# stefanopini/simple-HRNet

Hardware: AMD Instinct MI355X
Metric: person-crops/sec HRNet-W48 384x288 (model forward + heat-map decode) (higher is better)
Workload: dtype bf16; 1 GPU; HRNet-W48 384x288, batch=256 random crops per GPU, bf16 MFMA (BASELINE configs[2]); global_batch=256, micro_batch=256, lanes_per_gpu=1, parallelism=dp1 (crop sharding, RCCL all-gather of keypoints), weights=random-init seeded (synth_state_dict seed 0), BN stats randomised, engine_switches=

## Files before the change

### include/hrnet_mi355.h

```cpp
#ifndef HRNET_MI355_H
#define HRNET_MI355_H

#include <stddef.h>
#include <stdint.h>

#ifdef __cplusplus
extern "C" {
#endif

typedef struct hrn_ctx *hrn_handle;

enum { HRN_F32 = 0, HRN_BF16 = 1, HRN_F16 = 2 };
enum { HRN_BOX_I32 = 0, HRN_BOX_F32 = 1 };
enum { HRN_T_F32 = 0, HRN_T_I64 = 1 };

typedef struct {
    const char *name;
    const void *data;
    int32_t ndim;
    int64_t dims[4];
    int32_t dtype;
} hrn_tensor_desc;

typedef struct {
// ... 168 lines not shown
int hrn_refine_coords(hrn_handle h, const float *heatmaps_dev, int n, int refine, float *coords_dev, void *stream);

int hrn_nms(int32_t *keep_out, int32_t *num_out, const float *boxes_host, int boxes_num, int boxes_dim,
            float nms_overlap_thresh, int device_id);
int hrn_nms_release(int device_id);
const char *hrn_nms_last_error(void);

int hrn_oks_nms(int32_t *keep_out, int32_t *num_out, const double *kpts, const double *areas, const int32_t *order, int n, int J,
                double thresh, const double *sigmas, double in_vis_thre);
int hrn_soft_oks_nms(int32_t *keep_out, int32_t *num_out, const double *kpts, const double *areas, const double *scores_sorted,
                     const int32_t *order, int n, int J, double thresh, const double *sigmas, double in_vis_thre);
int hrn_pose_similarity(const double *boxes_a, const float *poses_a, int na, const double *boxes_b, const float *poses_b, int nb, int J,
                        float *sim_bbox, float *sim_pose);
int hrn_assignment(const double *cost, int rows, int cols, int32_t *row_to_col);

typedef struct {
    char name[96];
    int32_t c, h, w;
    int32_t conv_index;
} hrn_tap_info;
int hrn_tap_count(hrn_handle h);
int hrn_get_tap_info(hrn_handle h, int index, hrn_tap_info *out);
int hrn_forward_tap(hrn_handle h, const void *images_dev, int n, const char *tap_name, int crop0, int ncrops, int crop_step,
                    float *dst_dev, float *heatmaps_dev, void *stream);

int hrn_conv_count(hrn_handle h);
int hrn_get_conv_info(hrn_handle h, int index, hrn_conv_info *out);
double hrn_flops_per_crop(hrn_handle h);
int64_t hrn_workspace_bytes(hrn_handle h);
int64_t hrn_map_rebuilds(hrn_handle h);
int hrn_launches_per_pass(hrn_handle h);
int hrn_stem_fused(hrn_handle h);
int hrn_conv_compact(hrn_handle h, int index);
const char *hrn_switches(hrn_handle h);
int64_t hrn_debug_pad_violations(hrn_handle h);
int hrn_plan_block_map(hrn_handle h, int group, int n, int reverse, int32_t *blocks, int capacity, int32_t *members,
                       int member_capacity);
int hrn_plan_direct_map(hrn_handle h, int group, int n, int32_t *blocks, int capacity, int32_t *members, int member_capacity,
                        int32_t *pixels_per_tile);
int hrn_plan_s2_map(hrn_handle h, int group, int n, int32_t *blocks, int capacity, int32_t *parts, int part_capacity,
                    int32_t *active);
int hrn_profile_pass(hrn_handle h, const void *images_dev, int n, float *conv_ms, int conv_ms_len,
                     float *other_ms , void *stream);
const char *hrn_version(void);

#ifdef __cplusplus
}
#endif
#endif
```

### simple-hrnet_amd/_lib.py

```python
from __future__ import annotations

import ctypes
import os
import shutil
import subprocess
from typing import List

_HERE = os.path.dirname(os.path.abspath(__file__))
CSRC = os.path.join(_HERE, "csrc")
INCLUDE = os.path.join(os.path.dirname(_HERE), "include")
LIB_PATH = os.path.join(_HERE, "libhrnet_mi355.so")
if os.environ.get("HRN_LIB_TAG"):
    LIB_PATH = LIB_PATH.replace(".so", "_%s.so" % os.environ["HRN_LIB_TAG"])
SOURCES = ["kernels.hip", "conv3x3_lds.hip", "conv_s2.hip", "stem_fused.hip", "conv3x3_f32.hip", "bottleneck_chain.hip", "prepath.hip", "warp.hip", "nms.hip", "postproc.cpp", "hrnet_mi355.cpp",
           "decode.hip",
           "score.hip",
           "draw.hip",
           "track.hip",
           "pose_nms.hip",
           "letterbox.hip",
           "assoc.hip",
           "conv3x3_lds_f16.hip", "conv_s2_f16.hip", "bottleneck_chain_f16.hip"]
HEADERS = [os.path.join(CSRC, "kernels.h"), os.path.join(CSRC, "dt16.h"), os.path.join(CSRC, "argmax.h"), os.path.join(CSRC, "conv3x3_n96.inc"), os.path.join(CSRC, "conv3x3_lds.inc"),
           os.path.join(CSRC, "conv_s2.inc"), os.path.join(CSRC, "bottleneck_chain.inc"), os.path.join(INCLUDE, "hrnet_mi355.h")]
# ... 208 lines not shown
    "hrn_crop_geometry": (ctypes.c_int, [_P, ctypes.c_int, ctypes.c_int, _P, ctypes.c_int, ctypes.c_int, ctypes.c_int, ctypes.c_int, _P, _P]),
    "hrn_crop_geometry_last_error": (ctypes.c_char_p, []),
    "hrn_pose_boxes": (ctypes.c_int, [_P, ctypes.c_int, ctypes.c_int, _P, ctypes.c_int, ctypes.c_float, ctypes.c_int, ctypes.c_double,
                                      ctypes.c_double, _P]),
    "hrn_pose_boxes_last_error": (ctypes.c_char_p, []),
    "hrn_boxes_from_poses": (ctypes.c_int, [_P, _P, ctypes.c_int, ctypes.c_int, _P, ctypes.c_int, ctypes.c_float, ctypes.c_int,
                                            ctypes.c_double, ctypes.c_double, _P, _P]),
    "hrn_preprocess_frames_dev": (ctypes.c_int, [_P, ctypes.POINTER(Frame), ctypes.c_int, _P, ctypes.c_int, _P, ctypes.c_int, ctypes.c_int,
                                                 _P, _P, _P, _P]),
    "hrn_preprocess_frames_yuv_dev": (ctypes.c_int, [_P, ctypes.POINTER(YuvFrameC), ctypes.c_int, _P, ctypes.c_int, _P, ctypes.c_int,
                                                     ctypes.c_int, _P, _P, _P, _P]),
    "hrn_forward_flip_tta": (ctypes.c_int, [_P, _P, ctypes.c_int, _P, ctypes.c_int, ctypes.c_int, _P, _P, _P, _P]),
    "hrn_forward_refined": (ctypes.c_int, [_P, _P, ctypes.c_int, _P, ctypes.c_int, ctypes.c_int, _P, _P, _P]),
    "hrn_refine_coords": (ctypes.c_int, [_P, _P, ctypes.c_int, ctypes.c_int, _P, _P]),
    "hrn_nms": (ctypes.c_int, [_P, _P, _P, ctypes.c_int, ctypes.c_int, ctypes.c_float, ctypes.c_int]),
    "hrn_nms_release": (ctypes.c_int, [ctypes.c_int]),
    "hrn_nms_last_error": (ctypes.c_char_p, []),
    "hrn_oks_nms": (ctypes.c_int, [_P, _P, _P, _P, _P, ctypes.c_int, ctypes.c_int, ctypes.c_double, _P, ctypes.c_double]),
    "hrn_soft_oks_nms": (ctypes.c_int, [_P, _P, _P, _P, _P, _P, ctypes.c_int, ctypes.c_int, ctypes.c_double, _P, ctypes.c_double]),
    "hrn_pose_similarity": (ctypes.c_int, [_P, _P, ctypes.c_int, _P, _P, ctypes.c_int, ctypes.c_int, _P, _P]),
    "hrn_assignment": (ctypes.c_int, [_P, ctypes.c_int, ctypes.c_int, _P]),
    "hrn_tap_count": (ctypes.c_int, [_P]),
    "hrn_get_tap_info": (ctypes.c_int, [_P, ctypes.c_int, ctypes.POINTER(TapInfo)]),
    "hrn_forward_tap": (ctypes.c_int, [_P, _P, ctypes.c_int, ctypes.c_char_p, ctypes.c_int, ctypes.c_int, ctypes.c_int, _P, _P, _P]),
    "hrn_conv_count": (ctypes.c_int, [_P]),
    "hrn_get_conv_info": (ctypes.c_int, [_P, ctypes.c_int, ctypes.POINTER(ConvInfo)]),
    "hrn_flops_per_crop": (ctypes.c_double, [_P]),
    "hrn_workspace_bytes": (ctypes.c_int64, [_P]),
    "hrn_map_rebuilds": (ctypes.c_int64, [_P]),
    "hrn_launches_per_pass": (ctypes.c_int, [_P]),
    "hrn_switches": (ctypes.c_char_p, [_P]),
    "hrn_stem_fused": (ctypes.c_int, [_P]),
    "hrn_conv_compact": (ctypes.c_int, [_P, ctypes.c_int]),
    "hrn_debug_pad_violations": (ctypes.c_int64, [_P]),
    "hrn_plan_block_map": (ctypes.c_int, [_P, ctypes.c_int, ctypes.c_int, ctypes.c_int, _P, ctypes.c_int, _P, ctypes.c_int]),
    "hrn_plan_direct_map": (ctypes.c_int, [_P, ctypes.c_int, ctypes.c_int, _P, ctypes.c_int, _P, ctypes.c_int, _P]),
    "hrn_plan_s2_map": (ctypes.c_int, [_P, ctypes.c_int, ctypes.c_int, _P, ctypes.c_int, _P, ctypes.c_int, _P]),
    "hrn_profile_pass": (ctypes.c_int, [_P, _P, ctypes.c_int, ctypes.POINTER(ctypes.c_float), ctypes.c_int,
                                        ctypes.POINTER(ctypes.c_float), _P]),
    "hrn_version": (ctypes.c_char_p, []),
}

_lib = None


def load(auto_build: bool = True) -> ctypes.CDLL:
    global _lib
    if _lib is not None:
        return _lib
    if auto_build and needs_build():
        build()
    lib = ctypes.CDLL(LIB_PATH)
    for name, (res, args) in SYMBOLS.items():
        fn = getattr(lib, name)
        fn.restype = res
        fn.argtypes = args
    _lib = lib
    return lib


def header_symbols() -> List[str]:
    import re

    text = open(os.path.join(INCLUDE, "hrnet_mi355.h")).read()
    text = re.sub(r"/\*.*?\*/", "", text, flags=re.S)
    return sorted(set(re.findall(r"\b(hrn_[a-z_0-9]+)\s*\(", text)))
# ... 1 lines not shown
```

### simple-hrnet_amd/csrc/ctx_memory.inc

```
    bool hip_ok(hipError_t e, const char *what) {
        if (e == hipSuccess) return true;
        err = std::string(what) + ": " + hipGetErrorString(e);
        return false;
    }
    bool refuse_plan_only() {
        if (plan_only) err = "plan-only handle (device_id < 0): there is no CPU compute path";
        return plan_only;
    }

    bool allocate() {
        workspace_bytes = 0;
        for (auto &b : buffers) workspace_bytes += (int64_t)b.bytes;
        const int64_t small_crops = std::min<int64_t>(max_batch, (191 + head_slabs) / head_slabs);
        const int64_t part = std::max((int64_t)max_batch * joints * head_slabs, small_crops * joints * head_slabs_small);
        workspace_bytes += part * 8;
        if (plan_only) {
            fill_problems();
            index_s2groups();
            blob = (char *)calloc(1, (size_t)blob_bytes);
            return blob != nullptr;
        }
        if (!hip_ok(hipSetDevice(device), "hipSetDevice")) return false;
        for (auto &b : buffers) {
            if (!hip_ok(hipMalloc((void **)&b.dev, b.bytes), "hipMalloc(activation)")) return false;
// ... 110 lines not shown
                            ents.push_back({key, int2{prob | (nt << 8) | (tiles << 16), mt0 | (fused ? 1 << 29 : small_conv(cv) ? 1 << 30 : 0)}, bm});
                        }
            }
        }
        std::stable_sort(ents.begin(), ents.end(), [](const Ent &a, const Ent &b) { return a.key < b.key; });
        if (tile_px_out) {
            tile_px_out->resize(ents.size());
            for (size_t i = 0; i < ents.size(); ++i) (*tile_px_out)[i] = ents[i].bm;
        }
        if (out) {
            out->resize(ents.size());
            for (size_t i = 0; i < ents.size(); ++i) (*out)[i] = ents[i].v;
        }
        return (int)ents.size();
    }

    const Tensor &grid_of(const ConvOp &cv) const { return tensors[cv.up ? cv.in_t : cv.out_t]; }

    ConvArgs conv_args(const ConvOp &cv, int nb, bool rev) const {
        const Tensor &ti = tensors[cv.in_t], &to = grid_of(cv);
        ConvArgs a;
        a.in = row0(cv.in_t), a.out = row0(cv.out_t);
        a.w = blob + cv.w_off, a.bias = (const float *)(blob + cv.b_off);
        a.res = cv.res_t >= 0 ? row0(cv.res_t) : nullptr;
        a.cin = cv.cin, a.cout = cv.cout;
        a.in_wp = ti.wp, a.in_hpwp = ti.hpwp;
        a.out_h = to.h, a.out_w = to.w, a.out_wp = to.wp, a.out_hpwp = to.hpwp;
        a.m = nb * to.hpwp;
        a.ksize = cv.k, a.stride = cv.stride, a.relu = cv.relu, a.kchunks = cv.kchunks;
        a.rev = rev;
        a.pre_mode = pre_mode;
        a.wlds = direct_wlds && is16() ? 1 : 0;
        a.xlds = conv_xl(cv) ? 1 : 0;
        a.up = cv.up ? 1 : 0, a.up_a = cv.up ? (cv.up - 1) >> 1 : 0, a.up_b = cv.up ? (cv.up - 1) & 1 : 0;
        a.up_wp = tensors[cv.out_t].wp, a.up_hpwp = tensors[cv.out_t].hpwp;
        for (int t = 0; t < 4; ++t) {
            const int dy = (t >> 1) - 1 + a.up_a, dx = (t & 1) - 1 + a.up_b;
            a.taps[t] = cv.up ? dy * ti.wp + dx : 0;
        }
        return a;
    }

    int direct_group_blocks(const DirectGroup &g, int nb, std::vector<int2> *out, int mr = 4) const {
        struct Cls {
            int in_t, k, stride;
            std::vector<int> members;
            double cost = 0;
        };
        std::vector<Cls> cls;
        for (size_t k = 0; k < g.conv_idx.size(); ++k) {
            const ConvOp &cv = convs[g.conv_idx[k]];
            size_t ci = 0;
            for (; ci < cls.size(); ++ci)
                if (cls[ci].in_t == cv.in_t && cls[ci].k == cv.k && cls[ci].stride == cv.stride) break;
            if (ci == cls.size()) cls.push_back(Cls{cv.in_t, cv.k, cv.stride, {}, 0});
            cls[ci].members.push_back((int)k);
            cls[ci].cost += (double)grid_of(cv).hpwp * (cv.cout / (16 * g.nr)) * cv.kchunks;
        }
        std::stable_sort(cls.begin(), cls.end(), [](const Cls &a, const Cls &b) { return a.cost > b.cost; });
        int n = 0;
        if (out) out->clear();
        for (const Cls &cl : cls) {
            const int mtiles = (nb * grid_of(convs[g.conv_idx[cl.members[0]]]).hpwp + 64 * mr - 1) / (64 * mr);
            for (int round = 0; round * 8 < mtiles; ++round)
                for (int k : cl.members) {
                    const int ngroups = convs[g.conv_idx[k]].cout / (16 * g.nr);
// ... 297 lines not shown
```

### simple-hrnet_amd/csrc/ctx_run.inc

```
    struct Timing {
        std::vector<hipEvent_t> ev;
    };

    bool run_pass(const float *images, int nb, const void *boxes, int box_dtype, float *pts, float *heatmaps,
                  hipStream_t s, Timing *tm, int flip = 0, const TapReq *tap = nullptr, int refine = RF_NONE) {
        if (tm && !hip_ok(hipEventRecord(tm->ev[0], s), "hipEventRecord")) return false;
        const bool fused_stem = stem_fuse && !(tap && tap->op == 0);
        for (size_t oi = 0; oi < ops.size(); ++oi) {
            const bool rev = alternate && (oi & 1);
            hipError_t e = hipSuccess;
            if (fused_stem && oi == 0)
                e = exec_stem_fused(images, nb, s, flip);
            else if (!(fused_stem && (int)oi == stem_conv2_op))
                e = exec_op(ops[oi], rev, images, nb, boxes, box_dtype, pts, heatmaps, s, flip, refine);
            if (!hip_ok(e, "kernel launch")) return false;
            if (tap && tap->op == (int)oi) {
                const Tensor &t = tensors[tap->tensor];
                TapArgs a;
                a.in = row0(tap->tensor), a.dst = tap->dst;
                a.c = t.c, a.h = t.h, a.w = t.w, a.wp = t.wp, a.hpwp = t.hpwp;
                a.crop0 = tap->crop0, a.ncrops = tap->ncrops, a.crop_step = tap->crop_step;
                if (!hip_ok(launch_tap(dtype, a, s), "tap launch")) return false;
            }
            if (tm && !hip_ok(hipEventRecord(tm->ev[oi + 1], s), "hipEventRecord")) return false;
        }
        return true;
    }

    hipError_t exec_stem_fused(const float *images, int nb, hipStream_t s, int flip) {
        S2Group &g = stemf;
        bool hit;
        MapSlot *sl = find_slot(g.slot, nb, &hit);
        hipError_t e = slot_ready(sl, hit, s);
        if (e != hipSuccess) return e;
        if (!hit) {
            sl->nblocks = s2_blocks(g, nb, &g.map_host);
            if (sl->nblocks > g.map_capacity) return hipErrorInvalidValue;
            memcpy(sl->pin, g.map_host.data(), (size_t)sl->nblocks * sizeof(int2));
            e = hipMemcpyAsync(sl->dev, sl->pin, (size_t)sl->nblocks * sizeof(int2), hipMemcpyHostToDevice, s);
            if (e == hipSuccess) e = hipEventRecord(sl->landed, s);
// ... 22 lines not shown
            a.w = (const float *)(blob + stem_w_off), a.bias = (const float *)(blob + stem_b_off);
            a.wp = (is16() && !disable_stem_mfma) ? (const void *)(blob + stem_wp_off) : nullptr;
            a.n = nb, a.H = H, a.W = W;
            a.out_h = t.h, a.out_w = t.w, a.out_wp = t.wp, a.out_hpwp = t.hpwp;
            a.flip = flip;
            e = launch_stem(dtype, a, s);
            break;
        }
        case OP_STEM7: {
            const Tensor &t = tensors[stem_out_t];
            Stem7Args a;
            a.images = images, a.out = row0(stem_out_t);
            a.w = (const float *)(blob + stem_w_off), a.bias = (const float *)(blob + stem_b_off);
            a.wp = (is16() && !disable_stem_mfma) ? (const void *)(blob + stem_wp_off) : nullptr;
            a.n = nb, a.H = H, a.W = W;
            a.out_h = t.h, a.out_w = t.w, a.out_wp = t.wp, a.out_hpwp = t.hpwp;
            a.flip = flip;
            e = launch_stem7(dtype, a, s);
            break;
        }
        case OP_MAXPOOL: {
            const Tensor &ti = tensors[pool_in_t], &to = tensors[pool_out_t];
            PoolArgs a;
            a.in = row0(pool_in_t), a.out = row0(pool_out_t);
            a.c = to.c, a.n = nb, a.in_wp = ti.wp, a.in_hpwp = ti.hpwp;
            a.out_h = to.h, a.out_w = to.w, a.out_wp = to.wp, a.out_hpwp = to.hpwp;
            e = launch_maxpool(dtype, a, s);
            break;
        }
        case OP_CONV: {
            const ConvOp &cv = convs[op.idx];
            const ConvArgs a = conv_args(cv, nb, rev);
            e = launch_conv(dtype, a, cv.nr, s);
            break;
        }
        case OP_CONV3_GROUP: {
            Conv3Group &g = groups[op.idx];
            bool hit;
            MapSlot *sl = find_slot(g.slot, nb, &hit);
            if ((e = slot_ready(sl, hit, s)) != hipSuccess) break;
            if (!hit) {
                sl->nblocks = group_blocks(g, nb, &g.map_host, rev);
                if (sl->nblocks > g.map_capacity) {
                    e = hipErrorInvalidValue;
                    break;
                }
                memcpy(sl->pin, g.map_host.data(), (size_t)sl->nblocks * sizeof(int2));
                e = hipMemcpyAsync(sl->dev, sl->pin, (size_t)sl->nblocks * sizeof(int2), hipMemcpyHostToDevice, s);
                if (e == hipSuccess) e = hipEventRecord(sl->landed, s);
                if (e != hipSuccess) break;
                sl->nb = nb;
                ++map_builds;
            }
            e = (dtype == HRN_F16 ? launch_conv3x3_lds_f16 : launch_conv3x3_lds)(probs_dev + g.prob_first, sl->dev, sl->nblocks, nb,
                                                                             convs[g.conv_idx[0]].ks, convs[g.conv_idx[0]].nr, s);
            break;
        }
        case OP_CONV_GROUP: {
            DirectGroup &g = dgroups[op.idx];
            bool hit;
            MapSlot *sl = find_slot(g.slot, nb, &hit);
            if ((e = slot_ready(sl, hit, s)) != hipSuccess) break;
            if (!hit) {
                for (size_t k = 0; k < g.conv_idx.size(); ++k) sl->args_pin[k] = conv_args(convs[g.conv_idx[k]], nb, rev);
                sl->mr = 4;
                while (sl->mr > 1 && direct_group_blocks(g, nb, nullptr, sl->mr) < 512) sl->mr >>= 1;
// ... 146 lines not shown
```

### simple-hrnet_amd/csrc/hrnet_mi355.cpp

```cpp
#include "../../include/hrnet_mi355.h"

#include <hip/hip_runtime.h>

#include <algorithm>
#include <cmath>
#include <cstdio>
#include <cstdlib>
#include <cstring>
#include <map>
#include <memory>
#include <string>
#include <vector>

#include "assoc_math.h"
#include "letterbox_math.h"
#include "pose_nms_math.h"
#include "kernels.h"
#include "track_geometry.h"

namespace {
#include "ctx_types.h"
}

namespace {
// ... 30 lines not shown
    struct Chain {
        int conv3, conv1, ds;
        int conv2 = -1;
    };
    std::vector<Chain> chains;
    std::vector<TapPoint> taps;
    Conv3Problem *probs_dev = nullptr;
    std::vector<Op> ops;
    int stem_out_t = -1, head_in_t = -1;
    int64_t stem_w_off = 0, stem_b_off = 0, stem_wp_off = 0, head_w_off = 0, head_b_off = 0, head_wp_off = 0;

    int64_t blob_bytes = 0;
    char *blob = nullptr;
    bool weights_loaded = false;

    bool disable_lds = env_sw("HRN_DISABLE_LDS") != nullptr;
    bool assoc_no_assign = env_sw("HRN_ASSOC_NO_ASSIGN") != nullptr;
    bool disable_group = env_sw("HRN_DISABLE_GROUP") != nullptr;
    bool disable_dgroup = env_sw("HRN_DISABLE_DGROUP") != nullptr;
    bool disable_chain = env_sw("HRN_DISABLE_CHAIN") != nullptr;
    bool small_tiles = env_sw("HRN_SMALL_TILES") ? atoi(env_sw("HRN_SMALL_TILES")) != 0 : true;
    int small_below = env_sw("HRN_SMALL_BELOW") ? atoi(env_sw("HRN_SMALL_BELOW")) : 384;
    int small_keep_above = env_sw("HRN_SMALL_KEEP") ? atoi(env_sw("HRN_SMALL_KEEP")) : 300;
    bool disable_chain_ds = env_sw("HRN_DISABLE_CHAIN_DS") != nullptr;
    int pre_mode = env_sw("HRN_PRE_MODE") ? atoi(env_sw("HRN_PRE_MODE")) : 1;
    int chain_blocks = env_sw("HRN_CHAIN_BLOCKS") ? atoi(env_sw("HRN_CHAIN_BLOCKS")) : 512;
    bool disable_chain3 = env_sw("HRN_DISABLE_CHAIN3") != nullptr;
    bool direct_wlds = !(env_sw("HRN_DIRECT_WLDS") && atoi(env_sw("HRN_DIRECT_WLDS")) == 0);
    bool direct_xlds = !(env_sw("HRN_DIRECT_XLDS") && atoi(env_sw("HRN_DIRECT_XLDS")) == 0);
    bool conv_xl(const ConvOp &cv) const {
        return direct_xlds && direct_wlds && is16() && cv.k == 3 && cv.stride == 2 && cv.cin % 32 == 0 && !cv.up && cv.res_t < 0 && cv.nr == 6 &&
               cv.kchunks >= 4;
    }
    bool disable_bbf = env_sw("HRN_BBF") && atoi(env_sw("HRN_BBF")) == 0;
    int bbf_tpb_div = env_sw("HRN_BBF_TPB_DIV") ? std::max(1, atoi(env_sw("HRN_BBF_TPB_DIV"))) : 3;
    double bbf_slide_cost = env_sw("HRN_BBF_SLIDE_COST") ? atof(env_sw("HRN_BBF_SLIDE_COST")) : 24600.0;
    int bbf_min_tiles = env_sw("HRN_BBF_MIN_TILES") ? atoi(env_sw("HRN_BBF_MIN_TILES")) : 1100;
    int dgroup_nr_mode = env_sw("HRN_DGROUP_NR") ? atoi(env_sw("HRN_DGROUP_NR")) : 1;
    bool disable_lds32 = env_sw("HRN_DISABLE_LDS32") != nullptr;
    bool disable_n96 = env_sw("HRN_DISABLE_N96") != nullptr;
    bool disable_fgroup = env_sw("HRN_DISABLE_FGROUP") != nullptr;
    bool disable_f32lds = env_sw("HRN_DISABLE_F32LDS") != nullptr;
    int f32_small_slices = env_sw("HRN_F32_SMALL_SLICES") ? atoi(env_sw("HRN_F32_SMALL_SLICES")) : 0;
    std::vector<Conv3Problem> probs_host;
    bool disable_compact = env_sw("HRN_DISABLE_COMPACT") != nullptr;
    double compact_min_pad = env_sw("HRN_COMPACT_MIN_PAD") ? atof(env_sw("HRN_COMPACT_MIN_PAD")) : 0.08;
    bool disable_s2 = env_sw("HRN_DISABLE_S2") != nullptr;
    int s2_min_tiles = env_sw("HRN_S2_MIN_TILES") ? atoi(env_sw("HRN_S2_MIN_TILES")) : 256;
    int s2_target_blocks = env_sw("HRN_S2_BLOCKS") ? std::max(1, atoi(env_sw("HRN_S2_BLOCKS"))) : 256;
    bool disable_stem_mfma = env_sw("HRN_DISABLE_STEM_MFMA") != nullptr;
    bool disable_stem_fuse = env_sw("HRN_DISABLE_STEM_FUSE") != nullptr;
    bool stem_fuse = false;
    int stem_conv2_op = -1;
    S2Group stemf;
    bool disable_head_mfma = env_sw("HRN_DISABLE_HEAD_MFMA") != nullptr;
    bool direct_nr6 = env_sw("HRN_DIRECT_NR6") ? atoi(env_sw("HRN_DIRECT_NR6")) != 0 : true;
    int half_stages_per_block = env_sw("HRN_HALF_STAGES") ? atoi(env_sw("HRN_HALF_STAGES")) : 8;
    bool alternate = env_sw("HRN_ALTERNATE") ? atoi(env_sw("HRN_ALTERNATE")) != 0 : true;
    int block_order = env_sw("HRN_BLOCK_ORDER") ? atoi(env_sw("HRN_BLOCK_ORDER")) : 1;
    int long_factor = env_sw("HRN_LONG_FACTOR") ? atoi(env_sw("HRN_LONG_FACTOR")) : 4;
    double long_share = env_sw("HRN_LONG_SHARE") ? atof(env_sw("HRN_LONG_SHARE")) : 0.85;
    int head_slabs = 1, head_slab_px = 1024;
    static constexpr int kHeadSlabPxSmall = 256;
    int head_slabs_small = 1;
    int head_px_for(int nb) const { return (long)nb * head_slabs >= 192 ? head_slab_px : kHeadSlabPxSmall; }
    int head_slabs_for(int nb) const { return (long)nb * head_slabs >= 192 ? head_slabs : head_slabs_small; }
// ... 1248 lines not shown
}

int hrn_conv_count(hrn_handle h) { return h ? (int)h->convs.size() : 0; }

int hrn_get_conv_info(hrn_handle h, int index, hrn_conv_info *out) {
    if (!h || !out || index < 0 || index >= (int)h->convs.size()) return 1;
    const ConvOp &cv = h->convs[index];
    memset(out, 0, sizeof *out);
    snprintf(out->name, sizeof out->name, "%s", cv.conv.c_str());
    out->cin = cv.cin, out->cout = cv.cout, out->ksize = cv.k, out->stride = cv.stride, out->relu = cv.relu;
    out->has_residual = cv.res_t >= 0;
    out->in_h = h->tensors[cv.in_t].h, out->in_w = h->tensors[cv.in_t].w;
    out->out_h = h->tensors[cv.out_t].h, out->out_w = h->tensors[cv.out_t].w;
    out->kpad = cv.kpad, out->nr = cv.nr, out->algo = cv.fuse_with >= 0 || cv.fused_away ? 2 : cv.n96 ? 3 : cv.s2 ? 4 : cv.algo, out->ks = cv.ks;
    out->w_offset = cv.w_off, out->w_bytes = cv.w_bytes, out->b_offset = cv.b_off;
    out->flops = cv.flops;
    return 0;
}

double hrn_flops_per_crop(hrn_handle h) {
    if (!h) return 0;
    double f = 2.0 * 64 * (h->model == 1 ? 147 : 27) * (h->H / 2) * (double)(h->W / 2);
    for (auto &cv : h->convs) f += cv.flops;
    f += 2.0 * h->joints * h->head_c * (h->H / 4) * (double)(h->W / 4);
    return f;
}

int64_t hrn_workspace_bytes(hrn_handle h) { return h ? h->workspace_bytes : 0; }
int64_t hrn_map_rebuilds(hrn_handle h) { return h ? h->map_builds : -1; }
int hrn_launches_per_pass(hrn_handle h) { return h ? (int)h->ops.size() - (h->stem_fuse ? 1 : 0) : 0; }
int hrn_stem_fused(hrn_handle h) { return h && h->stem_fuse ? 1 : 0; }
int hrn_conv_compact(hrn_handle h, int index) { return h && index >= 0 && index < (int)h->convs.size() && h->convs[index].compact ? 1 : 0; }
const char *hrn_switches(hrn_handle h) { return h ? h->switches.c_str() : ""; }

int64_t hrn_debug_pad_violations(hrn_handle h) {
    if (!h || h->plan_only) return -1;
    if (!h->hip_ok(hipSetDevice(h->device), "hipSetDevice")) return -1;
    unsigned long long *cnt = nullptr, host = 0;
    if (!h->hip_ok(hipMalloc((void **)&cnt, sizeof *cnt), "hipMalloc") || !h->hip_ok(hipMemset(cnt, 0, sizeof *cnt), "hipMemset")) return -1;
    bool ok = h->hip_ok(hipDeviceSynchronize(), "hipDeviceSynchronize");
    for (const Buffer &b : h->buffers) {
        if (!ok) break;
        PadCheckArgs a;
        a.buf = b.dev, a.count = cnt, a.rows = (long)b.rows, a.lead_rows = (long)b.lead_rows;
        a.c = b.c, a.h = b.h, a.w = b.w, a.wp = b.w + 1, a.hpwp = (b.h + 1) * (b.w + 1), a.nmax = h->max_batch;
        ok = h->hip_ok(launch_pad_check(h->dtype, a, nullptr), "pad check launch");
    }
    ok = ok && h->hip_ok(hipMemcpy(&host, cnt, sizeof host, hipMemcpyDeviceToHost), "hipMemcpy");
    (void)hipFree(cnt);
    return ok ? (int64_t)host : -1;
}

int hrn_plan_block_map(hrn_handle h, int group, int n, int reverse, int32_t *blocks, int capacity, int32_t *members, int member_capacity) {
    if (!h || n <= 0 || n > h->max_batch) return -1;
    if (group < 0 || group >= (int)h->groups.size()) return -1;
    const Conv3Group &g = h->groups[group];
    std::vector<int2> map;
    std::vector<int> px;
    const int nblocks = h->group_blocks(g, n, &map, reverse != 0, false, &px);
    for (int i = 0; i < nblocks && i < capacity; ++i) {
        const int x = map[i].x, y = map[i].y;
        int32_t *o = blocks + (size_t)i * 6;
        o[0] = x & 0xff, o[1] = (x >> 8) & 0xff, o[2] = x >> 16, o[3] = y & 0x1fffffff, o[4] = px[i],
        o[5] = ((y >> 29) & 1) | (((y >> 30) & 1) << 1);
    }
    int nm = 0;
// ... 121 lines not shown
```

### simple-hrnet_amd/csrc/kernels.h

```cpp
#pragma once
#include <hip/hip_runtime.h>
#include <stdint.h>

#include <atomic>
#include <cstdlib>
#include <cstring>

namespace hrn {

inline hipError_t set_dynamic_lds(const void *func, int bytes, std::atomic<unsigned long long> &done) {
    int dev = 0;
    hipError_t e = hipGetDevice(&dev);
    if (e != hipSuccess) return e;
    const unsigned long long bit = 1ull << (dev & 63);
    if (done.load(std::memory_order_acquire) & bit) return hipSuccess;
    e = hipFuncSetAttribute(func, hipFuncAttributeMaxDynamicSharedMemorySize, bytes);
    if (e == hipSuccess) done.fetch_or(bit, std::memory_order_release);
    return e;
}

inline const char *hrn_env(const char *name) {
    static const bool debug = [] {
        const char *v = getenv("HRN_DEBUG_ENV");
        return v && *v && strcmp(v, "0") != 0;
    }();
    return debug ? getenv(name) : nullptr;
}

enum { DT_F32 = 0, DT_BF16 = 1, DT_F16 = 2 };

struct ConvArgs {
    const void *in;
    void *out;
    const void *w;
    const float *bias;
    const void *res;
    int cin, cout;
    int in_wp, in_hpwp;
    int out_h, out_w, out_wp, out_hpwp;
    int m;
    int ksize, stride, relu;
    int kchunks;
    int rev;
    int pre_mode;
    int wlds;
    int xlds;
    int up, up_a, up_b, up_wp, up_hpwp;
    int taps[4];
};

struct Conv3Problem {
    const void *in;
    void *out;
    const void *w;
    const float *bias;
    const void *res;
    int cin, cout;
    int h, wd, wp, hpwp;
    int relu;
    int slices;
    int ntiles;
    int tiles_per_block;
    int bm;
    unsigned magic_hpwp, magic_wp;
    int shift_hpwp, shift_wp;
    const void *w2;
    const float *bias2;
    int n96;
    int compact, hw;
    unsigned magic_hw, magic_w;
    int shift_hw, shift_w;
    int slab_rows, slab_rows_small;
};
int conv3x3_n96_ch64();
int conv3x3_lds_bbf_ok(int wp);
int conv3x3_n96_max_rows();
int conv3x3_lds_bm(int ks, int nrb, int wp);
int conv3x3_f32_bm(int wp);
hipError_t launch_conv3x3_f32(const Conv3Problem *probs_dev, const void *blockmap_dev, int nblocks, int nb, int nrb, hipStream_t s);
// ... 312 lines not shown
    unsigned char pad[4];
    LetterboxFrame one;
    const LetterboxFrame *table;
    void *out;
};
hipError_t launch_letterbox(const LetterboxArgs &a, hipStream_t s);
struct DetFrame;
struct DetFilter;
struct DetArgs {
    int P, compact;
    const DetFrame *table;
    const float *dets;
    float *out;
    int *counts, *status;
};
hipError_t launch_detections_to_frame(const DetArgs &a, const DetFrame &one, const DetFilter &q, hipStream_t s);

struct TapArgs {
    const void *in;
    float *dst;
    int c, h, w, wp, hpwp, crop0, ncrops, crop_step;
};
hipError_t launch_tap(int dtype, const TapArgs &a, hipStream_t s);

struct PadCheckArgs {
    const void *buf;
    unsigned long long *count;
    long rows, lead_rows;
    int c, h, w, wp, hpwp, nmax;
};
hipError_t launch_pad_check(int dtype, const PadCheckArgs &a, hipStream_t s);

hipError_t launch_conv(int dtype, const ConvArgs &a, int nr, hipStream_t s);
hipError_t launch_conv_group(int dtype, const ConvArgs *probs_dev, const void *map_dev, int nblocks, int nr, int mr, int wlds,
                             hipStream_t s);
hipError_t launch_conv3x3_lds(const Conv3Problem *probs_dev, const void *blockmap_dev, int nblocks, int nb, int ks,
                              int nrb, hipStream_t s);
hipError_t launch_conv3x3_lds_f16(const Conv3Problem *probs_dev, const void *blockmap_dev, int nblocks, int nb, int ks,
                                  int nrb, hipStream_t s);
hipError_t launch_stem(int dtype, const StemArgs &a, hipStream_t s);
hipError_t launch_fuse(int dtype, const FuseArgs &a, hipStream_t s);
hipError_t launch_head(int dtype, const HeadArgs &a, hipStream_t s);

constexpr int kConvBlockRows = 704;

}
```

### simple-hrnet_amd/csrc/kernels.hip

```cpp
#include "kernels.h"
#include "argmax.h"
#include "dt16.h"
#include <stdlib.h>

namespace hrn {

typedef __attribute__((ext_vector_type(8))) __bf16 bf16x8;
typedef __attribute__((ext_vector_type(8))) short s16x8;
typedef __attribute__((ext_vector_type(4))) short s16x4;
typedef __attribute__((ext_vector_type(4))) float f32x4;

__device__ __forceinline__ float bf16_to_f32(unsigned short h) { return __uint_as_float(((unsigned)h) << 16); }
__device__ __forceinline__ unsigned short f32_to_bf16(float f) {
    unsigned u = __float_as_uint(f);
    u += 0x7fffu + ((u >> 16) & 1u);
    return (unsigned short)(u >> 16);
}

constexpr bool is16(int dt) { return dt != DT_F32; }

template <int DT>
struct Tr;
template <>
struct Tr<DT_BF16> {
// ... 328 lines not shown
    for (int i = 0; i < MR; ++i)
#pragma unroll
        for (int j = 0; j < NR; ++j) acc[i][j] = f32x4{0.f, 0.f, 0.f, 0.f};
    w_issue(0);
    px_issue(0);
    px_issue(1);
    for (int kc = 0; kc < kchunks; ++kc) {
        const int gi = kc / XL_G, c = kc - gi * XL_G;
        if (c == 0) {
            asm volatile("s_waitcnt vmcnt(%0)" ::"i"((XL_D - 1) * MR) : "memory");
            __builtin_amdgcn_s_barrier();
            w_issue(gi + 1);
        }
        px_issue(kc + XL_D - 1);
        asm volatile("s_waitcnt vmcnt(%0)" ::"i"((XL_D - 1) * MR + WOPS) : "memory");
        s16x8 a[MR], b[NR];
        const unsigned xa = xring + (kc % XL_D) * (MR * 1024) + lane16;
        const unsigned wa = lds0 + ((gi & 1) * NR * XL_G + c) * 1024 + lane16;
#pragma unroll
        for (int i = 0; i < MR; ++i) asm volatile("ds_read_b128 %0, %1 offset:%2" : "=v"(a[i]) : "v"(xa), "i"(i * 1024));
#pragma unroll
        for (int j = 0; j < NR; ++j) asm volatile("ds_read_b128 %0, %1 offset:%2" : "=v"(b[j]) : "v"(wa), "i"(j * XL_G * 1024));
        asm volatile("s_waitcnt lgkmcnt(0)" ::: "memory");
#pragma unroll
        for (int i = 0; i < MR; ++i)
#pragma unroll
            for (int j = 0; j < NR; ++j) acc[i][j] = mma<DT>(b[j], a[i], acc[i][j]);
    }
    asm volatile("s_waitcnt vmcnt(0)" ::: "memory");
    s16x8 rpre[1][1];
    conv_direct_epilogue<DT, NR, MR, false>(p, ng, m0, li, g, acc, rpre);
}

template <int DT, int NR, int MR, bool PRE, bool WL = false>
__global__ __launch_bounds__(256) void conv_direct_kernel(const ConvArgs p) {
    extern __shared__ __attribute__((aligned(16))) char smem_direct[];
    const int ngroups = p.cout / (16 * NR);
    const int ng = (blockIdx.x >> 3) % ngroups;
    const int mtile = (blockIdx.x / (8 * ngroups)) * 8 + (blockIdx.x & 7);
    if constexpr (WL && is16(DT) && NR == 6 && MR == 4 && !PRE) {
        if (p.xlds && conv_xl_ok(p)) {
            conv_direct_xl_body<DT, NR>(p, ng, mtile, smem_direct);
            return;
        }
    }
    conv_direct_body<DT, NR, MR, PRE, WL>(p, ng, mtile, smem_direct);
}

template <int DT, int NR, int MR, bool WL = false>
__global__ __launch_bounds__(256) void conv_direct_group_kernel(const ConvArgs *__restrict__ probs,
                                                                const int2 *__restrict__ map) {
    extern __shared__ __attribute__((aligned(16))) char smem_direct[];
    const int2 e = map[blockIdx.x];
    const int prob = __builtin_amdgcn_readfirstlane(e.x & 255), ng = __builtin_amdgcn_readfirstlane(e.x >> 8);
    const int mtile = __builtin_amdgcn_readfirstlane(e.y);
    const ConvArgs p = probs[prob];
    if constexpr (WL && is16(DT) && NR == 6 && MR == 4) {
        if (p.xlds && conv_xl_ok(p)) {
            conv_direct_xl_body<DT, NR>(p, ng, mtile, smem_direct);
            return;
        }
    }
    conv_direct_body<DT, NR, MR, false, WL>(p, ng, mtile, smem_direct);
}

template <int DT, int NR>
// ... 39 lines not shown
        if (nr == 3) return launch_conv_group_t<DT_F16, 3>(probs_dev, map, nblocks, mr, wlds, s);
        if (nr == 2) return launch_conv_group_t<DT_F16, 2>(probs_dev, map, nblocks, mr, wlds, s);
    } else {
        if (nr == 4) return launch_conv_group_t<DT_F32, 4>(probs_dev, map, nblocks, mr, wlds, s);
        if (nr == 3) return launch_conv_group_t<DT_F32, 3>(probs_dev, map, nblocks, mr, wlds, s);
        if (nr == 2) return launch_conv_group_t<DT_F32, 2>(probs_dev, map, nblocks, mr, wlds, s);
    }
    return hipErrorInvalidValue;
}

template <int DT, int NR, int MR, bool PRE>
static hipError_t launch_conv_tt(const ConvArgs &a, hipStream_t s) {
    const int mtiles = (a.m + 64 * MR - 1) / (64 * MR);
    dim3 grid(((mtiles + 7) / 8) * 8 * (a.cout / (16 * NR)));
    hipLaunchKernelGGL((conv_direct_kernel<DT, NR, MR, PRE>), grid, dim3(256), 0, s, a);
    return hipGetLastError();
}

template <int DT, int NR>
static hipError_t launch_conv_t(const ConvArgs &a, hipStream_t s) {
    if constexpr (is16(DT) && NR % 2 == 0) {
        const int pre_mode = a.pre_mode;
        if (a.res && a.ksize == 1 && pre_mode == 1) return launch_conv_tt<DT, NR, 4, true>(a, s);
        if (a.res && a.ksize == 1 && pre_mode == 2) return launch_conv_tt<DT, NR, 2, true>(a, s);
        if (a.res && a.ksize == 1 && pre_mode == 3) return launch_conv_tt<DT, NR, 2, false>(a, s);
    }
    const int ngroups = a.cout / (16 * NR);
    const long blocks4 = (long)((a.m + 255) / 256) * ngroups;
    if (blocks4 < 256) return launch_conv_tt<DT, NR, 1, false>(a, s);
    if (blocks4 < 512) return launch_conv_tt<DT, NR, 2, false>(a, s);
    if constexpr (is16(DT))
        if (a.wlds && a.kchunks >= 2 * WL_G) {
            const int mtiles = (a.m + 255) / 256;
            dim3 grid(((mtiles + 7) / 8) * 8 * (a.cout / (16 * NR)));
            const int lds = direct_lds_bytes<DT, NR>(a.xlds ? 2 : 1);
            static std::atomic<unsigned long long> lds_set{0};
            if (lds > 65536) {
                const hipError_t e = set_dynamic_lds((const void *)conv_direct_kernel<DT, NR, 4, false, true>, direct_lds_bytes<DT, NR>(2), lds_set);
                if (e != hipSuccess) return e;
            }
            hipLaunchKernelGGL((conv_direct_kernel<DT, NR, 4, false, true>), grid, dim3(256), lds, s, a);
            return hipGetLastError();
        }
    return launch_conv_tt<DT, NR, 4, false>(a, s);
}

hipError_t launch_conv(int dtype, const ConvArgs &a, int nr, hipStream_t s) {
    if (a.m <= 0) return hipSuccess;
    if (dtype == DT_BF16) {
        if (nr == 6) return launch_conv_t<DT_BF16, 6>(a, s);
        if (nr == 4) return launch_conv_t<DT_BF16, 4>(a, s);
        if (nr == 3) return launch_conv_t<DT_BF16, 3>(a, s);
        if (nr == 2) return launch_conv_t<DT_BF16, 2>(a, s);
    } else if (dtype == DT_F16) {
        if (nr == 6) return launch_conv_t<DT_F16, 6>(a, s);
        if (nr == 4) return launch_conv_t<DT_F16, 4>(a, s);
        if (nr == 3) return launch_conv_t<DT_F16, 3>(a, s);
        if (nr == 2) return launch_conv_t<DT_F16, 2>(a, s);
    } else {
        if (nr == 4) return launch_conv_t<DT_F32, 4>(a, s);
        if (nr == 3) return launch_conv_t<DT_F32, 3>(a, s);
        if (nr == 2) return launch_conv_t<DT_F32, 2>(a, s);
    }
    return hipErrorInvalidValue;
}

// ... 667 lines not shown
```

### simple-hrnet_amd/native.py

```python
from __future__ import annotations

import contextlib
import ctypes
import math
from typing import Dict, List, Optional, Sequence, Tuple, Union

import numpy as np
import torch

from . import _lib
from .frames import (PIX_FORMATS, YUV_MATRICES, YUV_RANGES, Frames, YuvFrame, _check_frame, _frame_kind, as_tensor,
                     device_tensor, frame_stack, host_array, host_bytes)
from .palettes import bgr_to_yuv_colors, embedded_palette, find_palette

DTYPES = {"fp32": 0, "f32": 0, "float32": 0, torch.float32: 0, "bf16": 1, "bfloat16": 1, torch.bfloat16: 1,
          "fp16": 2, "f16": 2, "float16": 2, "half": 2, torch.float16: 2}
DTYPE_NAMES = {0: "fp32", 1: "bf16", 2: "fp16"}
REFINE_MODES = {None: 0, "quarter": 1, "dark": 2}


def refine_code(refine) -> int:
    if not (refine is None or isinstance(refine, str)) or refine not in REFINE_MODES:
        raise ValueError("refine must be None, 'quarter' or 'dark', got %r" % (refine,))
    return REFINE_MODES[refine]
# ... 1000 lines not shown
        if info is None:
            raise KeyError("no tensor named %r is written by this plan" % name)
        dst = torch.empty((ncrops, info.c, info.h, info.w), dtype=torch.float32, device=x.device)
        h, w = self.resolution
        hm = torch.empty((n, self.nof_joints, h // 4, w // 4), dtype=torch.float32, device=x.device) if return_heatmaps else None
        self._launch("hrn_forward_tap", x.data_ptr(), n, name.encode(), int(crop0), int(ncrops), int(crop_step), dst.data_ptr(),
                     hm.data_ptr() if hm is not None else None)
        return (dst, hm) if return_heatmaps else dst

    def conv_infos(self) -> List[_lib.ConvInfo]:
        out = []
        for i in range(self._lib.hrn_conv_count(self._h)):
            ci = _lib.ConvInfo()
            rc = self._lib.hrn_get_conv_info(self._h, i, ctypes.byref(ci))
            self._check(rc, "hrn_get_conv_info")
            out.append(ci)
        return out

    def flops_per_crop(self) -> float:
        return float(self._lib.hrn_flops_per_crop(self._h))

    def workspace_bytes(self) -> int:
        return int(self._lib.hrn_workspace_bytes(self._h))

    def map_rebuilds(self) -> int:
        return int(self._lib.hrn_map_rebuilds(self._h))

    def launches_per_pass(self) -> int:
        return int(self._lib.hrn_launches_per_pass(self._h))

    def conv_compact(self, index: int) -> bool:
        return bool(self._lib.hrn_conv_compact(self._h, index))

    def stem_fused(self) -> bool:
        return bool(self._lib.hrn_stem_fused(self._h))

    def pad_violations(self) -> int:
        return int(self._lib.hrn_debug_pad_violations(self._h))

    def switches(self) -> str:
        return self._lib.hrn_switches(self._h).decode()

    def profile_pass(self, images: torch.Tensor):
        x = self._images_ptr(images)
        n = min(x.shape[0], self.max_batch)
        nconv = self._lib.hrn_conv_count(self._h)
        conv_ms = (ctypes.c_float * nconv)()
        other = (ctypes.c_float * 4)()
        self._launch("hrn_profile_pass", x.data_ptr(), n, conv_ms, nconv, other)
        return list(conv_ms), dict(zip(("stem", "fuse", "head", "decode"), list(other)))


class MultiDeviceHRNet:

    def __init__(self, devices: Sequence[int], c: int = 48, nof_joints: int = 17, resolution: Tuple[int, int] = (384, 288),
                 dtype="bf16", max_batch: int = 32, model_name: str = "HRNet"):
        from concurrent.futures import ThreadPoolExecutor

        if len(devices) < 1:
            raise ValueError("at least one device")
        self.devices = [int(d) for d in devices]
        self.nets = [NativeHRNet(c, nof_joints, resolution, dtype, max_batch=max_batch, device=d, model_name=model_name)
                     for d in self.devices]
        self.streams = [torch.cuda.Stream(torch.device("cuda", d)) for d in self.devices]
        self.pool = ThreadPoolExecutor(max_workers=len(self.devices), thread_name_prefix="hrn-dev")
        first = self.nets[0]
# ... 155 lines not shown
```

Before: 11790 crops/s.

## Add wide 512-thread direct conv kernel for stride-2 XL convs

Adds a direct-convolution kernel for stride-2 3x3 convs with cout divisible by 192. Each 512-thread block covers two channel groups, so each staged pixel tile feeds twice the output channels. Weights are double-buffered and a three-stage pixel ring is prefetched two stages ahead. It is on by default and can be disabled with an env switch. It adds counters and query APIs, and trades more LDS per block and lower occupancy for more input reuse.

New measurement: 11840 crops/s (median of 6 runs). Within noise of the previous version (+0.5%).

```diff
diff --git a/include/hrnet_mi355.h b/include/hrnet_mi355.h
--- a/include/hrnet_mi355.h
+++ b/include/hrnet_mi355.h
@@ -224,6 +224,9 @@
 int hrn_launches_per_pass(hrn_handle h);
 int hrn_stem_fused(hrn_handle h);
 int hrn_conv_compact(hrn_handle h, int index);
+int hrn_conv_xl_wide(hrn_handle h, int index);
+int hrn_conv_op_index(hrn_handle h, int index);
+int64_t hrn_xl_wide_launches(hrn_handle h);
 const char *hrn_switches(hrn_handle h);
 int64_t hrn_debug_pad_violations(hrn_handle h);
 int hrn_plan_block_map(hrn_handle h, int group, int n, int reverse, int32_t *blocks, int capacity, int32_t *members,
diff --git a/simple-hrnet_amd/_lib.py b/simple-hrnet_amd/_lib.py
--- a/simple-hrnet_amd/_lib.py
+++ b/simple-hrnet_amd/_lib.py
@@ -264,6 +264,9 @@
     "hrn_switches": (ctypes.c_char_p, [_P]),
     "hrn_stem_fused": (ctypes.c_int, [_P]),
     "hrn_conv_compact": (ctypes.c_int, [_P, ctypes.c_int]),
+    "hrn_conv_xl_wide": (ctypes.c_int, [_P, ctypes.c_int]),
+    "hrn_conv_op_index": (ctypes.c_int, [_P, ctypes.c_int]),
+    "hrn_xl_wide_launches": (ctypes.c_int64, [_P]),
     "hrn_debug_pad_violations": (ctypes.c_int64, [_P]),
     "hrn_plan_block_map": (ctypes.c_int, [_P, ctypes.c_int, ctypes.c_int, ctypes.c_int, _P, ctypes.c_int, _P, ctypes.c_int]),
     "hrn_plan_direct_map": (ctypes.c_int, [_P, ctypes.c_int, ctypes.c_int, _P, ctypes.c_int, _P, ctypes.c_int, _P]),
diff --git a/simple-hrnet_amd/csrc/ctx_memory.inc b/simple-hrnet_amd/csrc/ctx_memory.inc
--- a/simple-hrnet_amd/csrc/ctx_memory.inc
+++ b/simple-hrnet_amd/csrc/ctx_memory.inc
@@ -166,6 +166,7 @@
         a.pre_mode = pre_mode;
         a.wlds = direct_wlds && is16() ? 1 : 0;
         a.xlds = conv_xl(cv) ? 1 : 0;
+        a.xlw = conv_xlw(cv) ? 1 : 0;
         a.up = cv.up ? 1 : 0, a.up_a = cv.up ? (cv.up - 1) >> 1 : 0, a.up_b = cv.up ? (cv.up - 1) & 1 : 0;
         a.up_wp = tensors[cv.out_t].wp, a.up_hpwp = tensors[cv.out_t].hpwp;
         for (int t = 0; t < 4; ++t) {
diff --git a/simple-hrnet_amd/csrc/ctx_run.inc b/simple-hrnet_amd/csrc/ctx_run.inc
--- a/simple-hrnet_amd/csrc/ctx_run.inc
+++ b/simple-hrnet_amd/csrc/ctx_run.inc
@@ -6,6 +6,7 @@
                   hipStream_t s, Timing *tm, int flip = 0, const TapReq *tap = nullptr, int refine = RF_NONE) {
         if (tm && !hip_ok(hipEventRecord(tm->ev[0], s), "hipEventRecord")) return false;
         const bool fused_stem = stem_fuse && !(tap && tap->op == 0);
+        xlw_launches = 0;
         for (size_t oi = 0; oi < ops.size(); ++oi) {
             const bool rev = alternate && (oi & 1);
             hipError_t e = hipSuccess;
@@ -94,6 +95,7 @@
             const ConvOp &cv = convs[op.idx];
             const ConvArgs a = conv_args(cv, nb, rev);
             e = launch_conv(dtype, a, cv.nr, s);
+            if (conv_takes_xlw(a)) ++xlw_launches;
             break;
         }
         case OP_CONV3_GROUP: {
diff --git a/simple-hrnet_amd/csrc/hrnet_mi355.cpp b/simple-hrnet_amd/csrc/hrnet_mi355.cpp
--- a/simple-hrnet_amd/csrc/hrnet_mi355.cpp
+++ b/simple-hrnet_amd/csrc/hrnet_mi355.cpp
@@ -86,6 +86,9 @@
         return direct_xlds && direct_wlds && is16() && cv.k == 3 && cv.stride == 2 && cv.cin % 32 == 0 && !cv.up && cv.res_t < 0 && cv.nr == 6 &&
                cv.kchunks >= 4;
     }
+    bool direct_xlw = !(env_sw("HRN_DIRECT_XLW") && atoi(env_sw("HRN_DIRECT_XLW")) == 0);
+    bool conv_xlw(const ConvOp &cv) const { return direct_xlw && conv_xl(cv) && cv.cout % 192 == 0; }
+    int64_t xlw_launches = 0;
     bool disable_bbf = env_sw("HRN_BBF") && atoi(env_sw("HRN_BBF")) == 0;
     int bbf_tpb_div = env_sw("HRN_BBF_TPB_DIV") ? std::max(1, atoi(env_sw("HRN_BBF_TPB_DIV"))) : 3;
     double bbf_slide_cost = env_sw("HRN_BBF_SLIDE_COST") ? atof(env_sw("HRN_BBF_SLIDE_COST")) : 24600.0;
@@ -1400,6 +1403,16 @@
 int hrn_stem_fused(hrn_handle h) { return h && h->stem_fuse ? 1 : 0; }
 int hrn_conv_compact(hrn_handle h, int index) { return h && index >= 0 && index < (int)h->convs.size() && h->convs[index].compact ? 1 : 0; }
 const char *hrn_switches(hrn_handle h) { return h ? h->switches.c_str() : ""; }
+int hrn_conv_op_index(hrn_handle h, int index) {
+    if (!h) return -1;
+    for (size_t oi = 0; oi < h->ops.size(); ++oi)
+        if (h->ops[oi].kind == OP_CONV && h->ops[oi].idx == index) return (int)oi;
+    return -1;
+}
+int hrn_conv_xl_wide(hrn_handle h, int index) {
+    return hrn_conv_op_index(h, index) >= 0 && h->conv_xlw(h->convs[index]) ? 1 : 0;
+}
+int64_t hrn_xl_wide_launches(hrn_handle h) { return h ? h->xlw_launches : -1; }
 
 int64_t hrn_debug_pad_violations(hrn_handle h) {
     if (!h || h->plan_only) return -1;
diff --git a/simple-hrnet_amd/csrc/kernels.h b/simple-hrnet_amd/csrc/kernels.h
--- a/simple-hrnet_amd/csrc/kernels.h
+++ b/simple-hrnet_amd/csrc/kernels.h
@@ -45,6 +45,7 @@
     int pre_mode;
     int wlds;
     int xlds;
+    int xlw;
     int up, up_a, up_b, up_wp, up_hpwp;
     int taps[4];
 };
@@ -423,6 +424,7 @@
 hipError_t launch_pad_check(int dtype, const PadCheckArgs &a, hipStream_t s);
 
 hipError_t launch_conv(int dtype, const ConvArgs &a, int nr, hipStream_t s);
+bool conv_takes_xlw(const ConvArgs &a);
 hipError_t launch_conv_group(int dtype, const ConvArgs *probs_dev, const void *map_dev, int nblocks, int nr, int mr, int wlds,
                              hipStream_t s);
 hipError_t launch_conv3x3_lds(const Conv3Problem *probs_dev, const void *blockmap_dev, int nblocks, int nb, int ks,
diff --git a/simple-hrnet_amd/csrc/kernels.hip b/simple-hrnet_amd/csrc/kernels.hip
--- a/simple-hrnet_amd/csrc/kernels.hip
+++ b/simple-hrnet_amd/csrc/kernels.hip
@@ -384,6 +384,115 @@
     conv_direct_epilogue<DT, NR, MR, false>(p, ng, m0, li, g, acc, rpre);
 }
 
+constexpr int XLW_S = 3;
+constexpr int xlw_lds_bytes(int nr) { return 2 * XL_G * 2 * nr * 1024 + 4 * XLW_S * XL_G * 4 * 1024; }
+template <int DT, int NR>
+__device__ __forceinline__ void conv_direct_xlw_body(const ConvArgs &p, const int ngp, const int mtile_in, char *smem) {
+    constexpr int MR = 4, PH = MR / 2;
+    const int lane = threadIdx.x & 63, wave = __builtin_amdgcn_readfirstlane(threadIdx.x >> 6);
+    const int pg = wave >> 1, cg = wave & 1;
+    const int li = lane & 15, g = lane >> 4;
+    if (mtile_in * 64 * MR >= p.m) return;
+    const int mtile = p.rev ? (p.m + 64 * MR - 1) / (64 * MR) - 1 - mtile_in : mtile_in;
+    const int m0 = (mtile * 4 + pg) * (16 * MR);
+    const int cin = p.cin, in_wp = p.in_wp, kchunks = p.kchunks;
+    const int spt = cin >> 5;
+    const int guard = (in_wp + 1) * cin;
+    const GLOBAL_AS char *const base = (const GLOBAL_AS char *)p.in - (size_t)guard * 2;
+    unsigned xoff[PH];
+#pragma unroll
+    for (int u = 0; u < PH; ++u) {
+        const int q = m0 + (cg * PH + u) * 16 + li;
+        int r = 0;
+        if (q < p.m) {
+            const int n = q / p.out_hpwp, rem = q - n * p.out_hpwp;
+            const int ho = rem / p.out_wp, wo = rem - ho * p.out_wp;
+            r = n * p.in_hpwp + 2 * ho * in_wp + 2 * wo;
+        }
+        xoff[u] = ((unsigned)r * (unsigned)cin + (unsigned)(guard + g * 8)) * 2u;
+    }
+    constexpr int WST = 2 * NR * XL_G;
+    const unsigned lds0 = (unsigned)(size_t)(__attribute__((address_space(3))) char *)smem;
+    const unsigned xring = lds0 + 2 * WST * 1024 + pg * (XLW_S * XL_G * MR * 1024);
+    const GLOBAL_AS char *const wsrc = (const GLOBAL_AS char *)p.w + (size_t)(2 * ngp) * NR * kchunks * 1024;
+    const unsigned lane16 = lane * 16;
+    auto px_issue = [&](int st) {
+        const int slot = st % XLW_S;
+#pragma unroll
+        for (int c = 0; c < XL_G; ++c) {
+            const int kc = st * XL_G + c;
+            const int kq = kc < kchunks ? kc : kchunks - 1;
+            const int tap = kq / spt, sl = kq - tap * spt;
+            const int dh = (tap * 11) >> 5, dw = tap - dh * 3;
+            const GLOBAL_AS char *sb = base + ((long)((dh - 1) * in_wp + (dw - 1)) * cin + sl * 32) * 2;
+#pragma unroll
+            for (int u = 0; u < PH; ++u) xl_glds(sb, xoff[u], xring + ((slot * XL_G + c) * MR + cg * PH + u) * 1024);
+        }
+    };
+    static_assert(WST % 8 == 0, "weight pieces per wave");
+    constexpr int WOPS = WST / 8;
+    auto w_issue = [&](int gi) {
+#pragma unroll
+        for (int u = 0; u < WOPS; ++u) {
+            const int t = wave + 8 * u;
+            const int f = t / XL_G;
+            int c = gi * XL_G + (t - f * XL_G);
+            if (c >= kchunks) c = kchunks - 1;
+            xl_glds(wsrc + (size_t)(f * kchunks + c) * 1024, lane16, lds0 + ((gi & 1) * WST + t) * 1024);
+        }
+    };
+    f32x4 acc[MR][NR];
+#pragma unroll
+    for (int i = 0; i < MR; ++i)
+#pragma unroll
+        for (int j = 0; j < NR; ++j) acc[i][j] = f32x4{0.f, 0.f, 0.f, 0.f};
+    w_issue(0);
+    px_issue(0);
+    px_issue(1);
+    const int nst = (kchunks + XL_G - 1) / XL_G;
+    for (int st = 0; st < nst; ++st) {
+        asm volatile("s_waitcnt vmcnt(%0)" ::"i"(XL_G * PH) : "memory");
+        __builtin_amdgcn_s_barrier();
+        w_issue(st + 1);
+        px_issue(st + 2);
+#pragma unroll
+        for (int c = 0; c < XL_G; ++c) {
+            if (st * XL_G + c >= kchunks) break;
+            s16x8 a[MR], b[NR];
+            const unsigned xa = xring + ((st % XLW_S) * XL_G + c) * (MR * 1024) + lane16;
+            const unsigned wa = lds0 + ((st & 1) * WST + cg * NR * XL_G + c) * 1024 + lane16;
+#pragma unroll
+            for (int i = 0; i < MR; ++i) asm volatile("ds_read_b128 %0, %1 offset:%2" : "=v"(a[i]) : "v"(xa), "i"(i * 1024));
+#pragma unroll
+            for (int j = 0; j < NR; ++j) asm volatile("ds_read_b128 %0, %1 offset:%2" : "=v"(b[j]) : "v"(wa), "i"(j * XL_G * 1024));
+            static_assert(MR == 4 && NR == 6, "operands of the wait");
+            asm volatile("s_waitcnt lgkmcnt(0)"
+                         : "+v"(a[0]), "+v"(a[1]), "+v"(a[2]), "+v"(a[3]), "+v"(b[0]), "+v"(b[1]), "+v"(b[2]), "+v"(b[3]), "+v"(b[4]), "+v"(b[5])
+                         :
+                         : "memory");
+#pragma unroll
+            for (int i = 0; i < MR; ++i)
+#pragma unroll
+                for (int j = 0; j < NR; ++j) acc[i][j] = mma<DT>(b[j], a[i], acc[i][j]);
+        }
+    }
+    asm volatile("s_waitcnt vmcnt(0)" ::: "memory");
+    s16x8 rpre[1][1];
+    conv_direct_epilogue<DT, NR, MR, false>(p, 2 * ngp + cg, m0, li, g, acc, rpre);
+}
+
+template <int DT>
+__global__ __launch_bounds__(512) void conv_direct_xlw_kernel(const ConvArgs p) {
+    extern __shared__ __attribute__((aligned(16))) char smem_direct[];
+    const int ngroups = p.cout / (2 * 16 * 6);
+    const int ngp = (blockIdx.x >> 3) % ngroups;
+    const int mtile = (blockIdx.x / (8 * ngroups)) * 8 + (blockIdx.x & 7);
+    conv_direct_xlw_body<DT, 6>(p, ngp, mtile, smem_direct);
+}
+bool conv_takes_xlw(const ConvArgs &a) {
+    return a.xlw && a.xlds && a.wlds && !a.res && a.kchunks >= 2 * WL_G && (long)((a.m + 255) / 256) * (a.cout / 96) >= 512;
+}
+
 template <int DT, int NR, int MR, bool PRE, bool WL = false>
 __global__ __launch_bounds__(256) void conv_direct_kernel(const ConvArgs p) {
     extern __shared__ __attribute__((aligned(16))) char smem_direct[];
@@ -489,6 +598,15 @@
     if constexpr (is16(DT))
         if (a.wlds && a.kchunks >= 2 * WL_G) {
             const int mtiles = (a.m + 255) / 256;
+            if constexpr (NR == 6)
+                if (conv_takes_xlw(a)) {
+                    dim3 grid(((mtiles + 7) / 8) * 8 * (a.cout / (2 * 16 * NR)));
+                    static std::atomic<unsigned long long> lds_set{0};
+                    const hipError_t e = set_dynamic_lds((const void *)conv_direct_xlw_kernel<DT>, xlw_lds_bytes(NR), lds_set);
+                    if (e != hipSuccess) return e;
+                    hipLaunchKernelGGL((conv_direct_xlw_kernel<DT>), grid, dim3(512), xlw_lds_bytes(NR), s, a);
+                    return hipGetLastError();
+                }
             dim3 grid(((mtiles + 7) / 8) * 8 * (a.cout / (16 * NR)));
             const int lds = direct_lds_bytes<DT, NR>(a.xlds ? 2 : 1);
             static std::atomic<unsigned long long> lds_set{0};
diff --git a/simple-hrnet_amd/native.py b/simple-hrnet_amd/native.py
--- a/simple-hrnet_amd/native.py
+++ b/simple-hrnet_amd/native.py
@@ -1056,6 +1056,15 @@
     def conv_compact(self, index: int) -> bool:
         return bool(self._lib.hrn_conv_compact(self._h, index))
 
+    def conv_xl_wide(self, index: int) -> bool:
+        return bool(self._lib.hrn_conv_xl_wide(self._h, index))
+
+    def conv_op_index(self, index: int) -> int:
+        return int(self._lib.hrn_conv_op_index(self._h, index))
+
+    def xl_wide_launches(self) -> int:
+        return int(self._lib.hrn_xl_wide_launches(self._h))
+
     def stem_fused(self) -> bool:
         return bool(self._lib.hrn_stem_fused(self._h))
 
```
